# RManLuo/MAMDR

Hardware: AMD Instinct MI355X
Metric: domain-steps/sec (higher is better)
Workload: dtype f32; 1 GPU; mlp_meta_mamdr Taobao-10 bs=1024 (frozen pretrained tables); global_batch=1024, domains=10, step_definition=one MAMDR meta-epoch (DN + DR phases, all outer updates), parallelism=single GPU

## Files before the change

mamdr_amd/csrc/env_registry.h:

```cpp
#pragma once

namespace mamdr {

struct EnvSwitch {
    const char* name;
    const char* reader;
    const char* effect;
};

static const EnvSwitch kEnvSwitches[] = {
    {"MAMDR_DENSE_ADAM", "lib,bench", "1: per-step dense sweep of trainable tables instead of the lazy replay (same bits)"},
    {"MAMDR_LAZY_FLUSH_EVERY", "lib", "steps between forced replays of lagging table rows (default 32)"},
    {"MAMDR_LAZY_LOG_CAP", "lib", "capacity of the alpha ring of the lazy table Adam (tests: force it to wrap)"},
    {"MAMDR_NO_TAILFUSE", "lib", "1: the table kernels as launches of their own instead of riders"},
    {"MAMDR_TOWER_TILE", "lib,bench", "rows per tower workgroup: 0 automatic, 4, 16 (initial value of mamdr_set_tower_tile)"},
    {"MAMDR_FUSED", "lib", "0: slab path everywhere; 2: k_wgrad_adam path for every batch size (default: up to 4 rows x CUs)"},
    {"MAMDR_DM_EACH", "lib", "1: k_dm_finish after every step (diagnostic; same bits)"},
    {"MAMDR_DM_CALL", "lib", "1: k_dm_finish closes every call (diagnostic; same bits)"},
    {"MAMDR_T4_NO_W1L", "lib", "1: k_tower4 without the W1 image in LDS (diagnostic)"},
    {"MAMDR_NO_W2_DIRECT", "lib", "1: k_transpose_w opens a call instead of the W2-in-place tower instance"},
    {"MAMDR_NO_PREGATHER", "lib,bench", "1: no k_pass_prep; the tower gathers its rows itself"},
    {"MAMDR_NO_PREGATHER_RIDE", "lib", "1: no rider workgroups in k_wgrad_adam; every pass window is gathered by k_pass_prep_multi (same bits)"},
    {"MAMDR_FZ_S_INORDER", "lib", "1: S workgroup b of k_wgrad_adam takes column block b of dz1 instead of one its XCD's tiles read (A/B switch; same bits)"},
    {"MAMDR_STAR_DENSE_SLICES", "lib", "1: every per-domain Star slice swept every step (diagnostic; same bits)"},
    {"MAMDR_REC_CHUNK", "lib,tests", "candidates per pass of mamdr_recommend's phases (default 16384; rounded up to 64; tests: several chunks at tiny sizes; same bits)"},
    {"MAMDR_GRAPH_NO_DEFER", "lib", "1: a pair of weight-gradient launches per layer instead of the queued flat grid"},
    {"MAMDR_GRAPH_TILE32_BELOW", "lib", "row count below which the 32 x 32 GEMM tile is used (0: 64 x 64 everywhere)"},
    {"MAMDR_GRAPH_NO_TAIL_OPT", "lib", "1: k_graph_adam as a launch of its own (same bits)"},
    {"MAMDR_LIB_PATH", "host,bench", "load this build of the library instead of mamdr_amd/libmamdr_hip.so (tools/build_variant.sh)"},
    {"MAMDR_LANES", "host", "lanes per process (overrides train.lanes)"},
    {"MAMDR_SHARE_GPU", "host", "1: every rank of run.py on device 0 over gloo (testing on a 1-GPU box)"},
    {"MAMDR_COMM_TIMEOUT", "host", "seconds: process-group timeout of run.py"},
    {"MAMDR_TAIL_SYNC", "host", "sum: tensors outside theta / phi combined by sum instead of the step-weighted mean"},
    {"MAMDR_NO_PASS_WINDOW", "host", "1: every call gathers its own pass (no k_pass_prep_multi windows)"},
    {"MAMDR_PASS_WINDOW_ROWS", "host", "row budget of a pass window"},
    {"MAMDR_PNN_ENGINE", "host", "graph: PNN on the generic-layer engine (default: step kernels)"},
    {"MAMDR_NFM_ENGINE", "host", "graph: NFM on the generic-layer engine"},
    {"MAMDR_STAR_ENGINE", "host", "graph: Star's PartitionedNorm + StarFCN form on the generic-layer engine (default: step kernels)"},
    {"MAMDR_BENCH_*", "bench", "bench.py knobs: _BATCH _ROW_SCALE _DN_MODE _NO_PREFETCH _PREP_TIMING _PREWARM_S _SHARE_GPU _COMM_TIMEOUT _SKIP_<WORKLOAD>"},
    {"MAMDR_DIAG_FLAGS", "tools", "extra -D flags of the stamp tools' diagnostic builds"},
    {"MAMDR_STAMPS_PREBUILT", "tools", "stamp tools: use an already built variant"},
    {"MAMDR_DIST_AUC_SCALE", "tools", "row scale of tools/dist_auc.py"},
    {"MAMDR_TEST_*", "tests", "test-suite knobs: _ALL_CPUS _BLAS_THREADS _NO_ORACLE_POOL _NO_PINNING _REPORT_FRAC"},
};
constexpr int kNumEnvSwitches = (int)(sizeof(kEnvSwitches) / sizeof(kEnvSwitches[0]));

}
```

mamdr_amd/csrc/fused_kernels.hip:

```cpp
#include <hip/hip_ext.h>

#include "mamdr_kernels.h"
#include "wgrad_adam_deal.h"

namespace mamdr {

constexpr int FZ_THREADS = 512;
constexpr int FZ_WAVES = 8;
constexpr int FZ_RING = 32;
static_assert(FZ_SBLK == DM_PARTS && FZ_DEAL_EMB == EMB && FZ_DEAL_H1 == H1 && FZ_DEAL_H2 == H2 && FZ_DEAL_H3 == H3,
              "wgrad_adam_deal.h deals the tower of mamdr_device.h");
constexpr int FZ_OUTB = 2;
__host__ __device__ constexpr int fz_own_wgs(bool with_loss) { return FZ_SBLK + FZ_TILES + FZ_OUTB + (with_loss ? 1 : 0); }

#define FZSTAMP(k) MAMDR_STAMP(MAMDR_CYCLES, a.stamps && threadIdx.x == 0, a.stamps[blockIdx.x * 8 + (k)])
#define FZREAL(k) MAMDR_STAMP(MAMDR_REALTIME, a.stamps && threadIdx.x == 0, a.stamps[blockIdx.x * 8 + (k)])

__device__ __forceinline__ void fz_store(const FusedArgs& a, int e, float p, float m, float v) {
    if (a.optimizer == 2) {
        a.m[e] = m;
        return;
    }
    if (a.optimizer == 0) {
        a.m[e] = m;
        a.v[e] = v;
    }
    a.p[e] = p;
}

__device__ __forceinline__ void fz_share(int n_slots, int w, int& s0, int& s1) {
    const int per = (n_slots + FZ_WAVES - 1) / FZ_WAVES;
    s0 = min(w * per, n_slots);
    s1 = min(s0 + per, n_slots);
}

template <bool CSUM>
__device__ __forceinline__ void fz_dense(const float* __restrict__ A, int lda, const float* __restrict__ B, int ldb,
                                         int s0, int s1, f32x4 (&acc)[2], f32x2& csum) {
    const int lane = threadIdx.x & 63, j = lane & 15, kq = lane >> 4;
    const int n = s1 - s0;
    if (n <= 0) return;
    const unsigned aoff = (unsigned)(kq * lda + j), boff = (unsigned)(kq * ldb + 2 * j);
    const float* arow = A + (size_t)(4 * s0) * lda;
    const float* brow = B + (size_t)(4 * s0) * ldb;
    const size_t astep = (size_t)4 * lda, bstep = (size_t)4 * ldb;
    const int last = n - 1;
    float ra[FZ_RING];
    f32x2 rb[FZ_RING];
#pragma unroll
    for (int u = 0; u < FZ_RING; ++u) {
        const int idx = min(u, last);
        ra[u] = (arow + idx * astep)[aoff];
        rb[u] = *reinterpret_cast<const f32x2*>(brow + idx * bstep + boff);
    }
    __builtin_amdgcn_sched_barrier(0);
    const int passes = (n + FZ_RING - 1) / FZ_RING;
    int base = 0;
    for (int pass = 0; pass + 1 < passes; ++pass, base += FZ_RING) {
#pragma unroll
        for (int u = 0; u < FZ_RING; ++u) {
            acc[0] = MAMDR_MFMA16(ra[u], rb[u][0], acc[0]);
            acc[1] = MAMDR_MFMA16(ra[u], rb[u][1], acc[1]);
            if (CSUM) csum += rb[u];
            const int idx = min(base + u + FZ_RING, last);
            ra[u] = (arow + idx * astep)[aoff];
            rb[u] = *reinterpret_cast<const f32x2*>(brow + idx * bstep + boff);
// ... 18 lines not shown
    const int n = s1 - s0;
    if (n <= 0) return;
    const unsigned boff = (unsigned)(kq * ldb + (j & (FZ_SC - 1)));
    const int32_t* drow = domrow + 4 * s0;
    const float* brow = B + (size_t)(4 * s0) * ldb;
    const size_t bstep = (size_t)4 * ldb;
    const int last = n - 1;
    int rd[FZ_RING];
    float rb[FZ_RING];
#pragma unroll
    for (int u = 0; u < FZ_RING; ++u) {
        const int idx = min(u, last);
        rd[u] = (drow + idx * 4)[(unsigned)kq];
        rb[u] = (brow + idx * bstep)[boff];
    }
    __builtin_amdgcn_sched_barrier(0);
    const int passes = (n + FZ_RING - 1) / FZ_RING;
    int base = 0;
    for (int pass = 0; pass + 1 < passes; ++pass, base += FZ_RING) {
#pragma unroll
        for (int u = 0; u < FZ_RING; ++u) {
#pragma unroll
            for (int mt = 0; mt < MT; ++mt) {
                const float av = (rd[u] == 16 * mt + j) ? 1.0f : 0.0f;
                acc[mt] = MAMDR_MFMA16(av, rb[u], acc[mt]);
            }
            const int idx = min(base + u + FZ_RING, last);
            rd[u] = (drow + idx * 4)[(unsigned)kq];
            rb[u] = (brow + idx * bstep)[boff];
            __builtin_amdgcn_sched_barrier(0);
        }
    }
#pragma unroll
    for (int u = 0; u < FZ_RING; ++u) {
        const int dsel = (base + u < n) ? rd[u] : -1;
#pragma unroll
        for (int mt = 0; mt < MT; ++mt) {
            const float av = (dsel == 16 * mt + j) ? 1.0f : 0.0f;
            acc[mt] = MAMDR_MFMA16(av, rb[u], acc[mt]);
        }
        __builtin_amdgcn_sched_barrier(0);
    }
}

constexpr int FZ_RED = FZ_WAVES * 16 * 32;
constexpr int FZ_CS = FZ_RED;
constexpr int FZ_LDS_TILE = FZ_RED + FZ_WAVES * 32;
static int fz_lds_floats(int n_domain) {
    const int mt = (n_domain + 15) / 16;
    const int s = FZ_WAVES * 16 * mt * FZ_SC + 16 * mt * FZ_SC;
    return s > FZ_LDS_TILE ? s : FZ_LDS_TILE;
}

__device__ __forceinline__ void fz_tile_body(const FusedArgs& a, int t, float* lds) {
    const int tid = threadIdx.x, lane = tid & 63, j = lane & 15, kq = lane >> 4;
    const int w = __builtin_amdgcn_readfirstlane(tid >> 6);
    const FzTile ft = fz_tile(t);
    const int gemm = ft.gemm, ablk = ft.ablk, bblk = ft.bblk;
    const float* A;
    int lda, b_off, dst, ldn;
    if (gemm == 0) {
        A = a.xa + 16 * ablk;
        lda = a.xa_ld;
        b_off = 32 * bblk;
        ldn = H1;
        dst = a.L.w0 + 16 * ablk * H1 + 32 * bblk;
    } else if (gemm == 1) {
        A = a.acts + XDIM + 16 * ablk;
        lda = ACT_LD;
        b_off = H1 + 32 * bblk;
        ldn = H2;
        dst = a.L.w1 + 16 * ablk * H2 + 32 * bblk;
    } else {
        A = a.acts + XDIM + H1 + 16 * ablk;
        lda = ACT_LD;
        b_off = H1 + H2 + 32 * bblk;
        ldn = H3;
        dst = a.L.w2 + 16 * ablk * H3 + 32 * bblk;
    }
    const int em = tid >> 5, en = tid & 31;
    const int e = dst + em * ldn + en;
    const float p0 = a.p[e];
    const float m0 = a.optimizer == 1 ? 0.f : a.m[e];
    const float v0 = a.optimizer == 0 ? a.v[e] : 0.f;
    const bool bias_tile = gemm > 0 && ablk == 0;
    int be = 0;
    float bp0 = 0.f, bm0 = 0.f, bv0 = 0.f;
    if (bias_tile) {
        be = (gemm == 1 ? a.L.b1 + (b_off - H1) : a.L.b2 + (b_off - H1 - H2)) + (tid & 31);
        bp0 = a.p[be];
        bm0 = a.optimizer == 1 ? 0.f : a.m[be];
        bv0 = a.optimizer == 0 ? a.v[be] : 0.f;
    }
    int s0, s1;
    fz_share(a.rows_pad / 4, w, s0, s1);
    f32x4 acc[2] = {(f32x4){0.f, 0.f, 0.f, 0.f}, (f32x4){0.f, 0.f, 0.f, 0.f}};
    f32x2 csum = (f32x2){0.f, 0.f};
    FZSTAMP(1);
    if (bias_tile) fz_dense<true>(A, lda, a.dz + b_off, DZ_LD, s0, s1, acc, csum);
    else fz_dense<false>(A, lda, a.dz + b_off, DZ_LD, s0, s1, acc, csum);
#pragma unroll
    for (int r = 0; r < 4; ++r)
        *reinterpret_cast<f32x2*>(lds + (w * 16 + 4 * kq + r) * 32 + 2 * j) = (f32x2){acc[0][r], acc[1][r]};
    if (bias_tile) {
        csum[0] += __shfl_xor(csum[0], 16);
        csum[1] += __shfl_xor(csum[1], 16);
        csum[0] += __shfl_xor(csum[0], 32);
        csum[1] += __shfl_xor(csum[1], 32);
        if (lane < 16) *reinterpret_cast<f32x2*>(lds + FZ_CS + w * 32 + 2 * j) = csum;
    }
// ... 289 lines not shown
    return -1;
}
__device__ __forceinline__ void ride_resolve(const RideArgs& g, const RideArgs::Seg& s, int n_domain, int q, int& u, int& it) {
    const int64_t i = (int64_t)s.first + q;
    if (i < s.n) {
        int64_t src;
        prep_ids(s, g.n_user, g.n_item, i, src, u, it);
        prep_meta(s, n_domain, src, g.pdom + s.out_off, g.plabel + s.out_off, i);
    } else {
        prep_pad_meta(s, g.pdom + s.out_off, g.plabel + s.out_off, i);
        u = -1;
        it = 0;
    }
}
__device__ __forceinline__ void fz_ride_body(const FusedArgs& a, int r, float* lds) {
    const RideArgs& g = a.ride;
    const int tid = threadIdx.x, lane = tid & 63;
    const int w = __builtin_amdgcn_readfirstlane(tid >> 6);
    int* ids = reinterpret_cast<int*>(lds);
    if (tid < FZ_RIDE_ROWS) {
        const int q = r * FZ_RIDE_ROWS + tid;
        int u = -1, it = 0;
        if (q < g.seg[0].count) ride_resolve(g, g.seg[0], a.n_domain, q, u, it);
        else if (q - g.seg[0].count < g.seg[1].count) ride_resolve(g, g.seg[1], a.n_domain, q - g.seg[0].count, u, it);
        *reinterpret_cast<int2*>(ids + 2 * tid) = make_int2(u, it);
    }
    FZSTAMP(1);
    FZSTAMP(2);
    __syncthreads();
    FZSTAMP(3);
    constexpr int PER = FZ_RIDE_ROWS / FZ_WAVES;
    f32x4 v[PER];
    int us[PER];
#pragma unroll
    for (int k = 0; k < PER; ++k) {
        const int2 id = *reinterpret_cast<const int2*>(ids + 2 * (w * PER + k));
        us[k] = __builtin_amdgcn_readfirstlane(id.x);
        const int it = __builtin_amdgcn_readfirstlane(id.y);
        v[k] = *prep_src(g.user_tab, g.item_tab, max(us[k], 0), it, lane);
    }
#pragma unroll
    for (int k = 0; k < PER; ++k) {
        const int64_t row = ride_row(g, r * FZ_RIDE_ROWS + w * PER + k);
        if (row < 0) continue;
        if (us[k] >= 0) prep_store_row(g.xpre, row, lane, v[k]);
        else prep_pad_row(g.xpre, row, lane);
    }
    FZSTAMP(4);
}

__global__ __launch_bounds__(FZ_THREADS) void k_wgrad_adam(const FusedArgs a) {
    extern __shared__ __attribute__((aligned(16))) float lds[];
    const int b = (int)blockIdx.x;
    FZSTAMP(0);
    FZREAL(5);
    if (b < FZ_SBLK) fz_s_body(a, fz_s_block(b, (a.flags & FZ_F_S_INORDER) != 0), lds);
    else if (b < FZ_SBLK + FZ_TILES) fz_tile_body(a, b - FZ_SBLK, lds);
    else if (b < FZ_SBLK + FZ_TILES + FZ_OUTB) fz_out_body(a, b - FZ_SBLK - FZ_TILES, lds);
    else if (b < fz_own_wgs(a.loss_out != nullptr)) fz_loss_body(a, lds);
    else fz_ride_body(a, b - fz_own_wgs(a.loss_out != nullptr), lds);
    FZREAL(6);
}

int wgrad_adam_own_wgs(bool with_loss) { return fz_own_wgs(with_loss); }

void launch_wgrad_adam(const FusedArgs& a, hipStream_t s) {
    const int grid = fz_own_wgs(a.loss_out != nullptr) + a.ride.n_wg;
    const size_t lds = (size_t)fz_lds_floats(a.n_domain) * sizeof(float);
    if (lds > 65536) {
        static const bool big_lds_set = hipFuncSetAttribute(reinterpret_cast<const void*>(k_wgrad_adam),
                                                            hipFuncAttributeMaxDynamicSharedMemorySize,
                                                            (int)(fz_lds_floats(64) * sizeof(float))) == hipSuccess;
        (void)big_lds_set;
    }
    MAMDR_LAUNCH(k_wgrad_adam, dim3(grid), dim3(FZ_THREADS), lds, s, a);
}

__global__ __launch_bounds__(256) void k_dm_finish(const DmStep q, float* live_p, float* live_m, float* live_v) {
    const int i = blockIdx.x * 256 + threadIdx.x;
    if (i >= q.n_domain * (EMB / 4)) return;
    const int d = i / (EMB / 4), c4 = i - d * (EMB / 4);
    f32x4 p, m, v;
    dm_step4(q, d, c4, p, m, v);
    const size_t row = (size_t)d * EMB + 4 * c4;
    if (q.optimizer != 2) *reinterpret_cast<f32x4*>(live_p + row) = p;
    if (q.optimizer != 1) *reinterpret_cast<f32x4*>(live_m + row) = m;
    if (q.optimizer == 0) *reinterpret_cast<f32x4*>(live_v + row) = v;
}

void launch_dm_finish(const DmStep& q, float* live_p, float* live_m, float* live_v, hipStream_t s) {
    MAMDR_LAUNCH(k_dm_finish, dim3((q.n_domain * (EMB / 4) + 255) / 256), dim3(256), 0, s, q, live_p, live_m, live_v);
}

template <typename P>
__device__ __forceinline__ void pass_prep_row(const P& a, const float* user_tab, const float* item_tab, int n_user, int n_item,
                                              int n_domain, int64_t pos0, float* xpre, int32_t* pdom, float* plabel, int64_t i) {
    const int lane = threadIdx.x & 63;
    if (i >= a.n) {
        if (i < a.n + PREP_PAD) {
            prep_pad_row(xpre, i, lane);
            if (lane == 0) prep_pad_meta(a, pdom, plabel, i);
        }
        return;
    }
    int64_t src;
    int u, it;
    prep_ids(a, n_user, n_item, pos0 + i, src, u, it);
    const f32x4 v = *prep_src(user_tab, item_tab, u, it, lane);
    prep_store_row(xpre, i, lane, v);
    if (lane == 0) prep_meta(a, n_domain, src, pdom, plabel, i);
}
// ... 29 lines not shown
```

mamdr_amd/csrc/mamdr_api.hip:

```cpp
#include <hip/hip_runtime.h>

#include <cmath>
#include <cstdarg>
#include <cstdio>
#include <cstdlib>
#include <cstring>
#include <new>
#include <string>
#include <utility>
#include <vector>

#include "../../include/mamdr_hip.h"
#include "mamdr_kernels.h"
#include "env_registry.h"

using namespace mamdr;

namespace mamdr {
thread_local hipEvent_t g_prof_stop = nullptr;
}

namespace {

thread_local char g_err[512] = "";
// ... 59 lines not shown
    std::vector<SplitData> data;
    int64_t adam_t = 0;
    float b1p = 1.0f, b2p = 1.0f;
    uint32_t global_step = 0;
    int rows_pad_max = 0;
    float* acts = nullptr;
    float* dz = nullptr;
    float* dlogit = nullptr;
    float* w0dom_copy = nullptr;
    float* dm_copy = nullptr;
    bool lin_w0dom = false;
    float* wT = nullptr;
    bool fused = false;
    float* star_alpha = nullptr;
    int star_dense_slices = 0;
    int t4_no_w1l = 0;
    int fused_max_batch = 1024;
    int tower4_max_rows = 2048;
    float* pdm = nullptr;
    float* xpre = nullptr;
    int32_t* pdom = nullptr;
    float* plabel = nullptr;
    int64_t pre_cap = 0;
    struct PgEntry { int domain; const int32_t* perm; int64_t n, off; int batch; };
    std::vector<PgEntry> pg;
    size_t pg_pos = 0;
    int64_t pg_hits = 0;
    int64_t pg_launches = 0;
    float* xpre_ahead = nullptr;
    int32_t* pdom_ahead = nullptr;
    float* plabel_ahead = nullptr;
    int64_t pre_cap_ahead = 0;
    struct Ahead {
        bool on = false;
        std::vector<PgEntry> list;
        std::vector<int64_t> rows;
        PassPrepMultiArgs args;
        PrePlanCursor cur;
    } ahead;
    int n_cu = 0;
    bool ride_on = true;
    int64_t pg_rider_rows = 0;
    int64_t pg_remainder_rows = 0;
    bool use_pre = true;
    float* dmsnap[2] = {nullptr, nullptr};
    int dm_cur = 0;
    DmStep dm_pending{};
    bool dm_finish_call = false;
    bool wT_valid = false;
    bool w1t_unread = false;
    bool w2t_unread = false;
    int fused_flags = -1;
    bool fz_s_inorder = false;
    bool w2_direct_ok = true;
    bool dm_finish_each = false;
    int tower_tile = 0;
    float* dxe = nullptr;
    int32_t* urow = nullptr;
    int32_t* irow = nullptr;
    int32_t* map_u = nullptr;
    int32_t* map_i = nullptr;
    float* gbuf_u = nullptr;
    float* gbuf_i = nullptr;
    int32_t* hasdup_u = nullptr;
    int32_t* hasdup_i = nullptr;
    bool lazy = false;
    bool tables_dirty = false;
    int32_t* last_u = nullptr;
    int32_t* last_i = nullptr;
    float* alpha_log = nullptr;
    int log_cap = 1 << 16;
    int flush_every = 32;
    int64_t flush_t = 0;
    int64_t n_flush = 0;
    int64_t n_flush_forced = 0;
    float* fmq = nullptr;
    float* glin_u = nullptr;
    float* glin_i = nullptr;
    int32_t* domrow = nullptr;
    float* loss_part = nullptr;
    float* eval_part = nullptr;
    int64_t eval_part_cap = 0;
    float* slabs = nullptr;
    bool tail_fuse = true;
    int32_t* urow_alt = nullptr;
    int32_t* irow_alt = nullptr;
    int32_t* map_u_alt = nullptr;
    int32_t* map_i_alt = nullptr;
    bool rows_ready = false;
    bool catchup_ready = false;
    int slab_ld = 0;
    int s2_off = 0;
    TileDesc* tiles = nullptr;
    int n_tiles = 0;
    float* thresholds = nullptr;
    float* frozen_sumsq = nullptr;
    float* sumsq_partials = nullptr;
    int rec_chunk = 16384;
    int rec_cap = 0;
    float* rec_P = nullptr;
    float* rec_lin = nullptr;
    float* rec_q = nullptr;
    unsigned long long* rec_part = nullptr;
    unsigned long long* rec_best = nullptr;
#ifdef MAMDR_STAMPS
    unsigned long long* stamps = nullptr;
// ... 668 lines not shown
        q.out_off = p.out_off;
        q.n = (int)p.n;
        q.n_rows_split = (int)p.n_rows_split;
        q.first = (int)sl.seg[k].first;
        q.count = (int)sl.seg[k].count;
        q.pad_dom = p.pad_dom;
    }
    c->pg_rider_rows += sl.count();
}

static int fused_step(mamdr_ctx* c, const CallPlan& P, int64_t s, float alpha) {
    const int32_t optimizer = P.optimizer;
    const int64_t row_base = (P.first_step + s) * P.batch;
    const int rows = rows_at(P.pass_rows, row_base, P.batch);
    const int rows_pad = (int)pad_rows(rows);
    const bool use4 = takes_tower4(c, rows_pad);
    DmStep& dm_pending = c->dm_pending;
    float* const dense_m = (optimizer == MAMDR_OPT_ACCUMULATE ? c->accum : c->adam_m) + c->table_floats;
    TowerArgs ta;
    fill_step_tower(c, P, row_base, rows, ta);
    c->dm_cur ^= 1;
    ta.dms = dm_pending;
    ta.dm_hint = P.domain;
    if (P.pre) {
        const int64_t at = P.pre_base + row_base - P.pre_pos0;
        ta.xpre = c->xpre + (size_t)at * 2 * EMB;
        ta.pdom = c->pdom + at;
        ta.plabel = c->plabel + at;
    }
    ta.dm_live_p = c->params + c->table_floats + c->L.dm;
    ta.dm_live_m = dense_m + c->L.dm;
    ta.dm_live_v = c->adam_v + c->table_floats + c->L.dm;
    ta.dm_snap_out = c->dmsnap[c->dm_cur];
    ta.w2_direct = (P.w2_direct && (s == 0 || P.w2_all) && use4) ? 1 : 0;
    if (int rc = run_step_tower(c, ta, use4, s)) return rc;
    FusedArgs fa;
    memset(&fa, 0, sizeof(fa));
    fa.acts = c->acts;
    fa.dz = c->dz;
    fa.dlogit = c->dlogit;
    fa.domrow = c->domrow;
    fa.xa = ta.xpre ? ta.xpre : c->acts;
    fa.xa_ld = ta.xpre ? 2 * EMB : ACT_LD;
    fa.rows_pad = rows_pad;
    fa.rows = rows;
    fa.p = c->params + c->table_floats;
    fa.m = dense_m;
    fa.v = c->adam_v + c->table_floats;
    fa.L = c->L;
    fa.n_domain = c->cfg.n_domain;
    fa.dm_snap = c->dmsnap[c->dm_cur];
    fa.pdm = c->pdm;
    fa.wT = (P.need_wT && optimizer != MAMDR_OPT_ACCUMULATE) ? c->wT : nullptr;
    fa.flags = (c->w1t_unread ? FZ_F_W1T_UNREAD : 0) | (P.w2_all ? FZ_F_W2T_UNREAD : 0) | (c->fz_s_inorder ? FZ_F_S_INORDER : 0);
    c->fused_flags = fa.flags;
    fa.optimizer = optimizer;
    fa.alpha = alpha;
    fa.omb1 = P.omb1;
    fa.omb2 = P.omb2;
    fa.eps = c->cfg.adam_eps;
    fa.two_l2 = 2.0f * c->cfg.l2_emb;
    fa.loss_part = c->loss_part;
    fa.n_loss_tiles = use4 ? rows_pad / 4 : rows_pad / TILE_ROWS;
    fa.frozen_sumsq = c->frozen_sumsq;
    fa.l2_emb = c->cfg.l2_emb;
    fa.loss_out = P.loss_out ? P.loss_out + s : nullptr;
#ifdef MAMDR_STAMPS
    fa.stamps = c->stamps ? c->stamps + 65536 + (c->global_step & 1) * 4096 : nullptr;
#endif
    if (c->ahead.on && !c->profile) attach_riders(c, fa);
    {
        Prof p(c, MAMDR_KERNEL_WGRAD);
        launch_wgrad_adam(fa, c->stream);
    }
    dm_pending.snap = c->dmsnap[c->dm_cur];
    dm_pending.pdm = c->pdm;
    dm_pending.n_part = DM_PARTS;
    dm_pending.n_domain = c->cfg.n_domain;
    dm_pending.optimizer = optimizer;
    dm_pending.alpha = alpha;
    dm_pending.omb1 = P.omb1;
    dm_pending.omb2 = P.omb2;
    dm_pending.eps = c->cfg.adam_eps;
    dm_pending.two_l2 = 2.0f * c->cfg.l2_emb;
    if (c->dm_finish_each || (s + 1 == P.n_steps && (optimizer != MAMDR_OPT_ADAM || c->dm_finish_call))) finish_dm(c);
    c->global_step += 1;
    return MAMDR_OK;
}

static int slab_step(mamdr_ctx* c, const CallPlan& P, int64_t s, float alpha) {
    const SplitData& d = *P.d;
    const int32_t optimizer = P.optimizer;
    const float omb1 = P.omb1, omb2 = P.omb2;
    const int64_t row_base = (P.first_step + s) * P.batch;
    const int rows = rows_at(P.pass_rows, row_base, P.batch);
    const int rows_pad = (int)pad_rows(rows);
    const bool use4 = takes_tower4(c, rows_pad);
    if (c->cfg.emb_trainable && c->lazy && optimizer == MAMDR_OPT_ADAM)
        emb_pre_step(c, d, P.perm, row_base, rows, rows_pad, alpha, omb1, omb2);
    TowerArgs ta;
    fill_step_tower(c, P, row_base, rows, ta);
    if (int rc = run_step_tower(c, ta, use4, s)) return rc;

    if (c->cfg.emb_trainable && P.loss_out) {
        prof_break(c);
        launch_sumsq(c->params, (int64_t)c->cfg.n_user * EMB, c->sumsq_partials, c->frozen_sumsq + 0, c->stream);
        launch_sumsq(c->params + (size_t)c->cfg.n_user * EMB, (int64_t)c->cfg.n_item * EMB, c->sumsq_partials,
// ... 263 lines not shown
        ALLOC(c->irow_alt, rp * sizeof(int32_t));
        ALLOC(c->map_u_alt, (size_t)cfg->n_user * sizeof(int32_t));
        ALLOC(c->map_i_alt, (size_t)cfg->n_item * sizeof(int32_t));
        ALLOC(c->gbuf_u, rp * EMB * sizeof(float));
        ALLOC(c->gbuf_i, rp * EMB * sizeof(float));
        ALLOC(c->hasdup_u, rp * sizeof(int32_t));
        ALLOC(c->hasdup_i, rp * sizeof(int32_t));
        const char* dense_env = getenv("MAMDR_DENSE_ADAM");
        c->lazy = !(dense_env && atoi(dense_env) != 0);
        if (const char* fe = getenv("MAMDR_LAZY_FLUSH_EVERY")) c->flush_every = atoi(fe) > 0 ? atoi(fe) : c->flush_every;
        if (const char* cap_env = getenv("MAMDR_LAZY_LOG_CAP")) {
            const int cap = atoi(cap_env);
            if (cap >= 4 && (cap & (cap - 1)) == 0) c->log_cap = cap;
        }
        ALLOC(c->last_u, (size_t)cfg->n_user * sizeof(int32_t));
        ALLOC(c->last_i, (size_t)cfg->n_item * sizeof(int32_t));
        ALLOC(c->alpha_log, (size_t)c->log_cap * sizeof(float));
        if (c->deepfm) {
            ALLOC(c->glin_u, rp * sizeof(float));
            ALLOC(c->glin_i, rp * sizeof(float));
        }
    }
    if (c->deepfm || c->pnn) ALLOC(c->fmq, rp * EMB * sizeof(float));
    if (c->pnn) ALLOC(c->ipbuf, rp * 4 * sizeof(float));
    ALLOC(c->domrow, rp * sizeof(int32_t));
    ALLOC(c->loss_part, (rp / 4) * sizeof(float));
    ALLOC(c->wT, (size_t)WT_FLOATS * sizeof(float));
    {
        if (const char* nw = getenv("MAMDR_T4_NO_W1L")) c->t4_no_w1l = atoi(nw) != 0;
        {
            int dev = 0, n_cu = 0;
            if (hipGetDevice(&dev) != hipSuccess || hipDeviceGetAttribute(&n_cu, hipDeviceAttributeMultiprocessorCount, dev) != hipSuccess ||
                n_cu <= 0)
                n_cu = 256;
            c->n_cu = n_cu;
            const int one_round = std::min(2048, std::max(256, 4 * n_cu));
            c->fused_max_batch = one_round;
            if (cfg->tower == MAMDR_TOWER_MLP && !cfg->emb_trainable) c->tower4_max_rows = one_round;
        }
        const char* fe = getenv("MAMDR_FUSED");
        c->fused = cfg->tower == MAMDR_TOWER_MLP && !cfg->emb_trainable && !cfg->uncertainty_weight && c->lin_w0dom &&
                   cfg->n_domain <= 64 && !(fe && atoi(fe) == 0);
        if (c->fused && fe && atoi(fe) == 2) c->fused_max_batch = 1 << 30;
        if (c->fused) {
            ALLOC(c->pdm, (size_t)DM_PARTS * cfg->n_domain * EMB * sizeof(float));
            ALLOC(c->dmsnap[0], (size_t)3 * cfg->n_domain * EMB * sizeof(float));
            ALLOC(c->dmsnap[1], (size_t)3 * cfg->n_domain * EMB * sizeof(float));
            if (const char* de = getenv("MAMDR_DM_EACH")) c->dm_finish_each = atoi(de) != 0;
            if (const char* de = getenv("MAMDR_DM_CALL")) c->dm_finish_call = atoi(de) != 0;
            if (const char* de = getenv("MAMDR_NO_W2_DIRECT")) c->w2_direct_ok = atoi(de) == 0;
            if (const char* pe = getenv("MAMDR_NO_PREGATHER")) c->use_pre = atoi(pe) == 0;
            if (const char* pe = getenv("MAMDR_NO_PREGATHER_RIDE")) c->ride_on = atoi(pe) == 0;
            if (const char* se = getenv("MAMDR_FZ_S_INORDER")) c->fz_s_inorder = atoi(se) != 0;
        }
        c->w1t_unread = w1t_unread_now(c);
        c->w2t_unread = w2t_unread_now(c);
    }
    if (const char* ev = getenv("MAMDR_NO_TAILFUSE")) c->tail_fuse = atoi(ev) == 0;
    if (const char* ev = getenv("MAMDR_REC_CHUNK"))
        if (atoi(ev) > 0) c->rec_chunk = (int)std::min<int64_t>(((int64_t)atoi(ev) + REC_TILE - 1) / REC_TILE * REC_TILE, 1 << 20);
    ALLOC(c->slabs, (size_t)WGRAD_MAX_GROUPS * c->slab_ld * sizeof(float));
    ALLOC(c->tiles, tiles.size() * sizeof(TileDesc));
    ALLOC(c->thresholds, sizeof(thr));
    ALLOC(c->frozen_sumsq, 4 * sizeof(float));
    ALLOC(c->sumsq_partials, 1024 * sizeof(float));
#undef ALLOC
    hipError_t e = hipMemsetAsync(c->slabs, 0, (size_t)WGRAD_MAX_GROUPS * c->slab_ld * sizeof(float), c->stream);
    if (e == hipSuccess) e = hipMemsetAsync(c->frozen_sumsq, 0, 4 * sizeof(float), c->stream);
    if (cfg->emb_trainable) {
        if (e == hipSuccess) e = hipMemsetAsync(c->hasdup_u, 0, rp * sizeof(int32_t), c->stream);
        if (e == hipSuccess) e = hipMemsetAsync(c->hasdup_i, 0, rp * sizeof(int32_t), c->stream);
        if (e == hipSuccess) e = hipMemsetAsync(c->last_u, 0, (size_t)cfg->n_user * sizeof(int32_t), c->stream);
        if (e == hipSuccess) e = hipMemsetAsync(c->last_i, 0, (size_t)cfg->n_item * sizeof(int32_t), c->stream);
        if (e == hipSuccess) e = hipMemsetAsync(c->alpha_log, 0, (size_t)c->log_cap * sizeof(float), c->stream);
        launch_emb_map_init(c->map_u, cfg->n_user, c->stream);
        launch_emb_map_init(c->map_i, cfg->n_item, c->stream);
        launch_emb_map_init(c->map_u_alt, cfg->n_user, c->stream);
        launch_emb_map_init(c->map_i_alt, cfg->n_item, c->stream);
    }
    if (e == hipSuccess) e = hipMemcpyAsync(c->tiles, tiles.data(), tiles.size() * sizeof(TileDesc), hipMemcpyHostToDevice, c->stream);
    if (e == hipSuccess) e = hipMemcpyAsync(c->thresholds, thr, sizeof(thr), hipMemcpyHostToDevice, c->stream);
    if (e == hipSuccess) e = hipStreamSynchronize(c->stream);
    if (e != hipSuccess) {
        mamdr_destroy(c);
        return fail(MAMDR_EHIP, "workspace initialisation: %s", hipGetErrorString(e));
    }
    *out = c;
    return MAMDR_OK;
}

int mamdr_destroy(mamdr_ctx* c) {
    if (!c) return MAMDR_OK;
    for (int k = 0; k < MAMDR_KERNEL_COUNT; ++k)
        for (EventPair& p : c->ev[k]) {
            if (p.own_a) (void)hipEventDestroy(p.a);
            (void)hipEventDestroy(p.b);
        }
    for (hipEvent_t e : c->ev_pool) (void)hipEventDestroy(e);
    void* ptrs[] = {c->urow_alt, c->irow_alt, c->map_u_alt, c->map_i_alt, c->acts, c->dz, c->dlogit, c->w0dom_copy, c->dm_copy, c->wT, c->dxe, c->urow, c->irow, c->map_u, c->map_i, c->gbuf_u, c->gbuf_i, c->hasdup_u, c->hasdup_i, c->last_u, c->last_i, c->alpha_log, c->star_alpha, c->pdm, c->dmsnap[0], c->dmsnap[1], c->xpre, c->pdom, c->plabel, c->xpre_ahead, c->pdom_ahead, c->plabel_ahead, c->fmq, c->ipbuf, c->glin_u, c->glin_i, c->eff, c->pn, c->star_part, c->star_sums, c->star_dmpart, c->domrow, c->loss_part, c->eval_part, c->slabs,
                    c->rec_P, c->rec_lin, c->rec_q, c->rec_part, c->rec_best,
                    c->tiles, c->thresholds, c->frozen_sumsq, c->sumsq_partials};
    for (void* p : ptrs)
        if (p) (void)hipFree(p);
    delete c;
    return MAMDR_OK;
}
// ... 968 lines not shown
```

mamdr_amd/csrc/mamdr_kernels.h:

```cpp
#pragma once
#include <hip/hip_runtime.h>
#include <hip/hip_ext.h>
#include <stdint.h>

#include "mamdr_device.h"
#include "pregather_plan.h"

namespace mamdr {

struct OptArgsLite {
    int optimizer;
    float alpha;
    float omb1, omb2, eps;
    float two_l2;
};
constexpr int32_t EMB_UNTOUCHED = 0x7fffffff;

extern thread_local hipEvent_t g_prof_stop;
int env_warn_unknown();
#define MAMDR_LAUNCH(kernel, grid, block, lds, stream, ...)                                               \
    do {                                                                                                  \
        if (::mamdr::g_prof_stop) {                                                                       \
            hipExtLaunchKernelGGL(kernel, grid, block, lds, stream, nullptr, ::mamdr::g_prof_stop, 0, __VA_ARGS__); \
            ::mamdr::g_prof_stop = nullptr;                                                               \
// ... 341 lines not shown
}
__device__ __forceinline__ void dm_tile_writer(const TowerArgs& a, int tile, int n_tiles, int c, const float* parts,
                                               const DmTile& t) {
    const bool pend = a.dms.snap != nullptr;
    if (tile < a.n_domain) {
        float p = t.p, m = t.m, v = t.v;
        if (pend) dm_elem_finish(a.dms, c, parts + 2048, p, m, v);
        dm_store_elem(a, (size_t)tile * EMB + c, pend, p, m, v);
    }
    if (c < EMB / 4) {
        for (int d = tile + n_tiles; d < a.n_domain; d += n_tiles) {
            f32x4 p, m, v;
            const size_t row = (size_t)d * EMB + 4 * c, plane = (size_t)a.n_domain * EMB;
            if (pend) {
                dm_step4(a.dms, d, c, p, m, v);
                if (a.dms.optimizer != 2) *reinterpret_cast<f32x4*>(a.dm_live_p + row) = p;
                if (a.dms.optimizer != 1) *reinterpret_cast<f32x4*>(a.dm_live_m + row) = m;
                if (a.dms.optimizer == 0) *reinterpret_cast<f32x4*>(a.dm_live_v + row) = v;
            } else {
                p = *reinterpret_cast<const f32x4*>(a.dm_live_p + row);
                m = *reinterpret_cast<const f32x4*>(a.dm_live_m + row);
                v = *reinterpret_cast<const f32x4*>(a.dm_live_v + row);
            }
            *reinterpret_cast<f32x4*>(a.dm_snap_out + row) = p;
            *reinterpret_cast<f32x4*>(a.dm_snap_out + plane + row) = m;
            *reinterpret_cast<f32x4*>(a.dm_snap_out + 2 * plane + row) = v;
        }
    }
}

constexpr int FZ_RIDE_ROWS = 64;
constexpr int FZ_RIDE_CAP = 32;
struct RideArgs {
    const float* user_tab;
    const float* item_tab;
    float* xpre;
    int32_t* pdom;
    float* plabel;
    int n_user, n_item;
    int n_wg;
    struct Seg {
        const int32_t* uid;
        const int32_t* pid;
        const int32_t* dom;
        const float* label;
        const int32_t* perm;
        int64_t out_off;
        int n, n_rows_split, first, count, pad_dom;
    } seg[2];
};
constexpr int FZ_F_W1T_UNREAD = 1;
constexpr int FZ_F_W2T_UNREAD = 2;
constexpr int FZ_F_S_INORDER = 4;
struct FusedArgs {
    const float* acts;
    const float* dz;
    const float* dlogit;
    const int32_t* domrow;
    const float* xa;
    int xa_ld;
    int rows_pad, rows;
    float* p;
    float* m;
    float* v;
    DenseLayout L;
    int n_domain;
    const float* dm_snap;
    float* pdm;
    float* wT;
    int flags;
    int optimizer;
    float alpha, omb1, omb2, eps, two_l2;
    const float* loss_part;
    int n_loss_tiles;
    const float* frozen_sumsq;
    float l2_emb;
    float* loss_out;
    RideArgs ride;
#ifdef MAMDR_STAMPS
    unsigned long long* stamps;
#endif
};
void launch_wgrad_adam(const FusedArgs& a, hipStream_t s);
int wgrad_adam_own_wgs(bool with_loss);
struct PassPrepArgs {
    const float* user_tab;
    const float* item_tab;
    const int32_t* uid;
    const int32_t* pid;
    const int32_t* dom;
    const float* label;
    const int32_t* perm;
    int64_t pos0, n, n_rows_split;
    int n_user, n_item, n_domain;
    int pad_dom;
    float* xpre;
    int32_t* pdom;
    float* plabel;
    const float* tw_dense;
    DenseLayout tw_L;
    float* tw_wT;
    int n_prep_wgs;
};
constexpr int PREP_MAX_PASSES = 16;
struct PassPrepMultiArgs {
    const float* user_tab;
// ... 305 lines not shown
```

mamdr_amd/csrc/wgrad_adam_deal.h:

```cpp
#pragma once

#if defined(__HIPCC__) || defined(__CUDACC__)
#define MAMDR_DEAL_FN __host__ __device__ constexpr
#else
#define MAMDR_DEAL_FN constexpr
#endif

namespace mamdr {

constexpr int FZ_DEAL_EMB = 128, FZ_DEAL_H1 = 256, FZ_DEAL_H2 = 128, FZ_DEAL_H3 = 64;
constexpr int FZ_SBLK = 32;
constexpr int FZ_SC = 8;
constexpr int FZ_T0 = (2 * FZ_DEAL_EMB / 16) * (FZ_DEAL_H1 / 32);
constexpr int FZ_T1 = (FZ_DEAL_H1 / 16) * (FZ_DEAL_H2 / 32);
constexpr int FZ_T2 = (FZ_DEAL_H2 / 16) * (FZ_DEAL_H3 / 32);
constexpr int FZ_TILES = FZ_T0 + FZ_T1 + FZ_T2;

static_assert(FZ_SBLK % 8 == 0, "tile t and workgroup FZ_SBLK + t must share the residue mod 8");
static_assert(FZ_SBLK * FZ_SC == FZ_DEAL_H1 && FZ_SBLK == 32, "fz_s_block deals 32 blocks of 8 columns");
static_assert(FZ_TILES % 8 == 0, "the same number of tiles on every residue");

MAMDR_DEAL_FN int fz_s_block(int b, bool in_order) {
    return in_order ? b : 16 * ((b & 7) >> 2) + 4 * (b >> 3) + (b & 3);
}

struct FzTile {
    int gemm;
    int ablk;
    int bblk;
};
MAMDR_DEAL_FN FzTile fz_tile(int t) {
    const int x = t & 7, xa = x & 3, xb = x >> 2, li = t >> 3;
    if (li < 16) return FzTile{0, 4 * xa + (li & 3), 4 * xb + (li >> 2)};
    if (li < 24) return FzTile{1, 4 * xa + ((li - 16) & 3), 2 * xb + ((li - 16) >> 2)};
    return FzTile{2, 2 * xa + (li - 24), xb};
}

}
```

Measured before the change: 46570 domain-steps/s.

## Deal k_wgrad_adam workgroups to XCDs by matrix rectangle via constant table

Adds a compile-time deal table that decides which S block, GEMM tile, or output unit each workgroup of k_wgrad_adam handles. The new default groups each XCD (blockIdx mod 8) onto a contiguous rectangle of one weight matrix, so an XCD's L2 holds fewer distinct A/B operand blocks. The previous residue-mixed deal stays available behind MAMDR_FZ_DEAL_RESIDUE, and is also forced when MAMDR_FZ_S_INORDER is set. In exchange, each workgroup does one extra constant-memory load, and per-XCD work may end up less balanced.

```diff
diff --git a/mamdr_amd/csrc/env_registry.h b/mamdr_amd/csrc/env_registry.h
--- a/mamdr_amd/csrc/env_registry.h
+++ b/mamdr_amd/csrc/env_registry.h
@@ -21,6 +21,7 @@
     {"MAMDR_NO_W2_DIRECT", "lib", "1: k_transpose_w opens a call instead of the W2-in-place tower instance"},
     {"MAMDR_NO_PREGATHER", "lib,bench", "1: no k_pass_prep; the tower gathers its rows itself"},
     {"MAMDR_NO_PREGATHER_RIDE", "lib", "1: no rider workgroups in k_wgrad_adam; every pass window is gathered by k_pass_prep_multi (same bits)"},
+    {"MAMDR_FZ_DEAL_RESIDUE", "lib", "1: k_wgrad_adam deals every XCD the same mix of S blocks and tiles of all three matrices instead of one rectangle of one matrix (A/B switch; same bits)"},
     {"MAMDR_FZ_S_INORDER", "lib", "1: S workgroup b of k_wgrad_adam takes column block b of dz1 instead of one its XCD's tiles read (A/B switch; same bits)"},
     {"MAMDR_STAR_DENSE_SLICES", "lib", "1: every per-domain Star slice swept every step (diagnostic; same bits)"},
     {"MAMDR_REC_CHUNK", "lib,tests", "candidates per pass of mamdr_recommend's phases (default 16384; rounded up to 64; tests: several chunks at tiny sizes; same bits)"},
diff --git a/mamdr_amd/csrc/fused_kernels.hip b/mamdr_amd/csrc/fused_kernels.hip
--- a/mamdr_amd/csrc/fused_kernels.hip
+++ b/mamdr_amd/csrc/fused_kernels.hip
@@ -10,8 +10,9 @@
 constexpr int FZ_RING = 32;
 static_assert(FZ_SBLK == DM_PARTS && FZ_DEAL_EMB == EMB && FZ_DEAL_H1 == H1 && FZ_DEAL_H2 == H2 && FZ_DEAL_H3 == H3,
               "wgrad_adam_deal.h deals the tower of mamdr_device.h");
-constexpr int FZ_OUTB = 2;
-__host__ __device__ constexpr int fz_own_wgs(bool with_loss) { return FZ_SBLK + FZ_TILES + FZ_OUTB + (with_loss ? 1 : 0); }
+static_assert(FZ_OUTB == 2 && FZ_OWN == FZ_SBLK + FZ_TILES + FZ_OUTB, "two output-unit workgroups of 32 columns of h3");
+__host__ __device__ constexpr int fz_own_wgs(bool with_loss) { return FZ_OWN + (with_loss ? 1 : 0); }
+__constant__ const FzDealTable c_fz_deal = fz_deal_table_make();
 
 #define FZSTAMP(k) MAMDR_STAMP(MAMDR_CYCLES, a.stamps && threadIdx.x == 0, a.stamps[blockIdx.x * 8 + (k)])
 #define FZREAL(k) MAMDR_STAMP(MAMDR_REALTIME, a.stamps && threadIdx.x == 0, a.stamps[blockIdx.x * 8 + (k)])
@@ -136,10 +137,9 @@
     return s > FZ_LDS_TILE ? s : FZ_LDS_TILE;
 }
 
-__device__ __forceinline__ void fz_tile_body(const FusedArgs& a, int t, float* lds) {
+__device__ __forceinline__ void fz_tile_body(const FusedArgs& a, const FzTile ft, float* lds) {
     const int tid = threadIdx.x, lane = tid & 63, j = lane & 15, kq = lane >> 4;
     const int w = __builtin_amdgcn_readfirstlane(tid >> 6);
-    const FzTile ft = fz_tile(t);
     const int gemm = ft.gemm, ablk = ft.ablk, bblk = ft.bblk;
     const float* A;
     int lda, b_off, dst, ldn;
@@ -535,11 +535,14 @@
 __global__ __launch_bounds__(FZ_THREADS) void k_wgrad_adam(const FusedArgs a) {
     extern __shared__ __attribute__((aligned(16))) float lds[];
     const int b = (int)blockIdx.x;
+    const int2 dealt = *reinterpret_cast<const int2*>(c_fz_deal.code[min(b, FZ_OWN - 1)]);
     FZSTAMP(0);
     FZREAL(5);
-    if (b < FZ_SBLK) fz_s_body(a, fz_s_block(b, (a.flags & FZ_F_S_INORDER) != 0), lds);
-    else if (b < FZ_SBLK + FZ_TILES) fz_tile_body(a, b - FZ_SBLK, lds);
-    else if (b < FZ_SBLK + FZ_TILES + FZ_OUTB) fz_out_body(a, b - FZ_SBLK - FZ_TILES, lds);
+    const int code = (a.flags & FZ_F_DEAL_RESIDUE) ? dealt.y : dealt.x;
+    const int role = b < FZ_OWN ? fz_code_role(code) : -1;
+    if (role == FZ_ROLE_S) fz_s_body(a, (a.flags & FZ_F_S_INORDER) ? b : fz_code_x(code), lds);
+    else if (role >= 0 && role < 3) fz_tile_body(a, FzTile{role, fz_code_x(code), fz_code_y(code)}, lds);
+    else if (role == FZ_ROLE_OUT) fz_out_body(a, fz_code_x(code), lds);
     else if (b < fz_own_wgs(a.loss_out != nullptr)) fz_loss_body(a, lds);
     else fz_ride_body(a, b - fz_own_wgs(a.loss_out != nullptr), lds);
     FZREAL(6);
diff --git a/mamdr_amd/csrc/mamdr_api.hip b/mamdr_amd/csrc/mamdr_api.hip
--- a/mamdr_amd/csrc/mamdr_api.hip
+++ b/mamdr_amd/csrc/mamdr_api.hip
@@ -135,6 +135,7 @@
     bool w2t_unread = false;
     int fused_flags = -1;
     bool fz_s_inorder = false;
+    bool fz_deal_residue = false;
     bool w2_direct_ok = true;
     bool dm_finish_each = false;
     int tower_tile = 0;
@@ -909,7 +910,8 @@
     fa.dm_snap = c->dmsnap[c->dm_cur];
     fa.pdm = c->pdm;
     fa.wT = (P.need_wT && optimizer != MAMDR_OPT_ACCUMULATE) ? c->wT : nullptr;
-    fa.flags = (c->w1t_unread ? FZ_F_W1T_UNREAD : 0) | (P.w2_all ? FZ_F_W2T_UNREAD : 0) | (c->fz_s_inorder ? FZ_F_S_INORDER : 0);
+    fa.flags = (c->w1t_unread ? FZ_F_W1T_UNREAD : 0) | (P.w2_all ? FZ_F_W2T_UNREAD : 0) | (c->fz_s_inorder ? FZ_F_S_INORDER : 0) |
+               (c->fz_deal_residue || c->fz_s_inorder ? FZ_F_DEAL_RESIDUE : 0);
     c->fused_flags = fa.flags;
     fa.optimizer = optimizer;
     fa.alpha = alpha;
@@ -1279,6 +1281,7 @@
             if (const char* pe = getenv("MAMDR_NO_PREGATHER")) c->use_pre = atoi(pe) == 0;
             if (const char* pe = getenv("MAMDR_NO_PREGATHER_RIDE")) c->ride_on = atoi(pe) == 0;
             if (const char* se = getenv("MAMDR_FZ_S_INORDER")) c->fz_s_inorder = atoi(se) != 0;
+            if (const char* se = getenv("MAMDR_FZ_DEAL_RESIDUE")) c->fz_deal_residue = atoi(se) != 0;
         }
         c->w1t_unread = w1t_unread_now(c);
         c->w2t_unread = w2t_unread_now(c);
diff --git a/mamdr_amd/csrc/mamdr_kernels.h b/mamdr_amd/csrc/mamdr_kernels.h
--- a/mamdr_amd/csrc/mamdr_kernels.h
+++ b/mamdr_amd/csrc/mamdr_kernels.h
@@ -417,6 +417,7 @@
 constexpr int FZ_F_W1T_UNREAD = 1;
 constexpr int FZ_F_W2T_UNREAD = 2;
 constexpr int FZ_F_S_INORDER = 4;
+constexpr int FZ_F_DEAL_RESIDUE = 8;
 struct FusedArgs {
     const float* acts;
     const float* dz;
diff --git a/mamdr_amd/csrc/wgrad_adam_deal.h b/mamdr_amd/csrc/wgrad_adam_deal.h
--- a/mamdr_amd/csrc/wgrad_adam_deal.h
+++ b/mamdr_amd/csrc/wgrad_adam_deal.h
@@ -15,6 +15,8 @@
 constexpr int FZ_T1 = (FZ_DEAL_H1 / 16) * (FZ_DEAL_H2 / 32);
 constexpr int FZ_T2 = (FZ_DEAL_H2 / 16) * (FZ_DEAL_H3 / 32);
 constexpr int FZ_TILES = FZ_T0 + FZ_T1 + FZ_T2;
+constexpr int FZ_OUTB = FZ_DEAL_H3 / 32;
+constexpr int FZ_OWN = FZ_SBLK + FZ_TILES + FZ_OUTB;
 
 static_assert(FZ_SBLK % 8 == 0, "tile t and workgroup FZ_SBLK + t must share the residue mod 8");
 static_assert(FZ_SBLK * FZ_SC == FZ_DEAL_H1 && FZ_SBLK == 32, "fz_s_block deals 32 blocks of 8 columns");
@@ -36,4 +38,76 @@
     return FzTile{2, 2 * xa + (li - 24), xb};
 }
 
+constexpr int FZ_ROLE_S = 3, FZ_ROLE_OUT = 4;
+MAMDR_DEAL_FN int fz_code(int role, int x, int y) { return role | (x << 3) | (y << 8); }
+MAMDR_DEAL_FN int fz_code_role(int code) { return code & 7; }
+MAMDR_DEAL_FN int fz_code_x(int code) { return (code >> 3) & 31; }
+MAMDR_DEAL_FN int fz_code_y(int code) { return code >> 8; }
+
+MAMDR_DEAL_FN int fz_residue_code(int b, bool in_order) {
+    if (b < FZ_SBLK) return fz_code(FZ_ROLE_S, fz_s_block(b, in_order), 0);
+    if (b < FZ_SBLK + FZ_TILES) {
+        const FzTile f = fz_tile(b - FZ_SBLK);
+        return fz_code(f.gemm, f.ablk, f.bblk);
+    }
+    return fz_code(FZ_ROLE_OUT, b - FZ_SBLK - FZ_TILES, 0);
 }
+
+struct FzDeal2 {
+    int code[FZ_OWN];
+    int n[8];
+};
+MAMDR_DEAL_FN void fz_deal2_put(FzDeal2& d, int x, int code) {
+    d.code[8 * d.n[x] + x] = code;
+    d.n[x] += 1;
+}
+MAMDR_DEAL_FN void fz_deal2_rect(FzDeal2& d, int x, int gemm, int a0, int a1, int b0, int b1, int sa0 = 0, int sa1 = 0, int sb = -1) {
+    for (int bb = b0; bb < b1; ++bb)
+        for (int ab = a0; ab < a1; ++ab)
+            if (!(bb == sb && ab >= sa0 && ab < sa1)) fz_deal2_put(d, x, fz_code(gemm, ab, bb));
+}
+MAMDR_DEAL_FN void fz_deal2_s(FzDeal2& d, int x, int blk0, int blk1) {
+    for (int blk = blk0; blk < blk1; ++blk) fz_deal2_put(d, x, fz_code(FZ_ROLE_S, blk, 0));
+}
+MAMDR_DEAL_FN FzDeal2 fz_deal2_make() {
+    FzDeal2 d{};
+    fz_deal2_rect(d, 0, 1, 0, 8, 0, 4, 7, 8, 3);
+    fz_deal2_rect(d, 1, 1, 8, 16, 0, 4, 14, 16, 3);
+    fz_deal2_put(d, 1, fz_code(1, 7, 3));
+    fz_deal2_s(d, 2, 20, 32);
+    fz_deal2_rect(d, 2, 2, 0, 8, 0, 2);
+    fz_deal2_rect(d, 2, 0, 14, 16, 7, 8);
+    fz_deal2_s(d, 3, 0, 6);
+    fz_deal2_rect(d, 3, 0, 0, 8, 0, 3);
+    fz_deal2_s(d, 4, 6, 12);
+    fz_deal2_rect(d, 4, 0, 8, 16, 0, 3);
+    fz_deal2_s(d, 5, 12, 16);
+    fz_deal2_rect(d, 5, 0, 0, 8, 3, 6);
+    for (int ob = 0; ob < FZ_OUTB; ++ob) fz_deal2_put(d, 5, fz_code(FZ_ROLE_OUT, ob, 0));
+    fz_deal2_s(d, 6, 16, 20);
+    fz_deal2_rect(d, 6, 0, 8, 16, 3, 6);
+    fz_deal2_rect(d, 6, 1, 14, 16, 3, 4);
+    fz_deal2_rect(d, 7, 0, 0, 16, 6, 8, 14, 16, 7);
+    return d;
+}
+constexpr FzDeal2 FZ_DEAL2 = fz_deal2_make();
+MAMDR_DEAL_FN bool fz_deal2_full(const FzDeal2& d) {
+    for (int x = 0; x < 8; ++x)
+        if (d.n[x] != (FZ_OWN - x + 7) / 8) return false;
+    return true;
+}
+static_assert(fz_deal2_full(FZ_DEAL2), "the dealing by matrix must fill every residue's 30 / 31 own workgroups");
+
+struct FzDealTable {
+    int code[FZ_OWN][2];
+};
+MAMDR_DEAL_FN FzDealTable fz_deal_table_make() {
+    FzDealTable t{};
+    for (int b = 0; b < FZ_OWN; ++b) {
+        t.code[b][0] = FZ_DEAL2.code[b];
+        t.code[b][1] = fz_residue_code(b, false);
+    }
+    return t;
+}
+
+}
```

New measurement: 47320 domain-steps/s, median of 6. 1.02x the previous value.
